# Dane-ME/keypoint-detection

Measured on AMD Instinct MI355X. Metric: images/sec @ 256x192 COCO-17 (MultiPersonKeypointModel.forward, given boxes), higher is better.
Workload: dtype fp32; 1 GPU; C2: batch 64/GPU, 256x192x3, 1 box/img, heatmap head + soft-argmax decode; model=MultiPersonKeypointModel (MobileNetV3-Small+FPN, HeatmapHead), global_batch=64, height=256, width=192, persons=1, precision=split, parallelism=dp1, streams_per_gpu=1, gather=False, gather_pipelined=False

## Files before the change

include/kpd.h:

```cpp
#ifndef KPD_H_
#define KPD_H_

#include <stddef.h>
#include <stdint.h>

#ifdef __cplusplus
extern "C" {
#endif

#define KPD_OK 0
#define KPD_EINVAL (-1)
#define KPD_EHIP (-2)
#define KPD_ESTATE (-3)

#define KPD_PRECISION_FP32 0
#define KPD_PRECISION_MIXED 1
#define KPD_PRECISION_SPLIT 2

typedef struct kpd_plan kpd_plan;

const char* kpd_last_error(void);
const char* kpd_version(void);

int kpd_plan_create(int device, int in_channels, kpd_plan** out);
// ... 115 lines not shown
                              void* stream);

#define KPD_COORD_SMOOTH_L1 0
#define KPD_COORD_MSE 1
#define KPD_COORD_HUBER 2
int kpd_coord_loss(const float* heat, const float* gt, const float* vis, int planes, int H, int W, float temperature,
                   int loss_type, float pixel_weight_scale, float distance_threshold, float* coords, float* loss,
                   float* grad, void* stream);

int kpd_softargmax_backward(const float* heat, const float* grad_coords, int planes, int H, int W, float temperature,
                            float* grad_heat, void* stream);

int kpd_plan_set_streams(kpd_plan* plan, int n);

int kpd_plan_set_graphs(kpd_plan* plan, int enable);

int kpd_bench_conv16(int split, int N, int H, int W, int cin, int cout, int dbg, int iters, float* ms);

#define KPD_BUILD_DIAG 1
int kpd_build_flags(void);

int kpd_fpn0x_class_table(int* cls_ng, int* cls_g, int* cls_woff, int* blocks);


int kpd_heatmap_head(kpd_plan* plan, const float* x, int R, int H, int W, int parts, float* heat, float* ch_w,
                     float* sp_w, void* stream);

int kpd_keypoint_head(kpd_plan* plan, const float* x, int R, int H, int W, float* keypoints, float* visibility,
                      void* stream);

int kpd_backbone(kpd_plan* plan, const float* image, int B, int C, int H, int W, float* out0, float* out1,
                 float* out2, float* out3, void* stream);

int kpd_backbone_body(kpd_plan* plan, const float* image, int B, int C, int H, int W, float* feat0, float* feat1,
                      float* feat2, float* feat3, void* stream);

int kpd_backbone_fpn(kpd_plan* plan, const float* feat0, const float* feat1, const float* feat2, const float* feat3,
                     int B, const int* sizes, float* out0, float* out1, float* out2, float* out3, void* stream);

int kpd_roi_features(kpd_plan* plan, const float* image, int B, int C, int H, int W, const float* boxes, int P,
                     const int32_t* rows, int n, float* out, void* stream);

int kpd_channel_attention(kpd_plan* plan, const float* x, int B, int C, int H, int W, float* scores, int32_t* topk,
                          int k, float* selected, void* stream);

#define KPD_DECODE_ARGMAX 0
// ... 48 lines not shown
```

keypoint-detection_amd/csrc/conv_glds.hip:

```cpp
#include <algorithm>
#include <type_traits>

#include "kpd_common.h"
#include "kpd_kernels.h"
#include "conv_epilogue.h"
#include "kpd_dma.h"

namespace {

typedef _Float16 f16x8 __attribute__((ext_vector_type(8)));
typedef __attribute__((address_space(3))) void lds_void;

constexpr int BM = 256, NT = 512, ROWB = 128;
constexpr unsigned OOB = 0x80000000u;

__device__ __forceinline__ void stamp16(unsigned long long* st, int i, unsigned long long v = 0, int row = -1) {
  if (st && threadIdx.x == 0)
    st[(size_t)(row < 0 ? blockIdx.x : row) * 8 + i] = v ? v : __builtin_amdgcn_s_memrealtime();
}

__device__ __forceinline__ float dpp_xor1(float x) {
  return __int_as_float(__builtin_amdgcn_mov_dpp(__float_as_int(x), 0xB1, 0xF, 0xF, true));
}
__device__ __forceinline__ float dpp_xor2(float x) {
// ... 846 lines not shown
}

constexpr int HP = kHmPitch, HPP = kHmRoiPos;
constexpr int HMS = 56;
constexpr int AWIN = 384;
template <int BMH>
constexpr int hm_awin() { return BMH + 128 <= AWIN ? AWIN : BMH + 128; }
template <int BMH>
constexpr int hm_epi_parts() { return BMH > 256 ? 2 : 1; }
template <int CIN, bool SPLIT>
constexpr int hm_nab() { return (CIN > 0 && (SPLIT ? CIN * 4 : CIN * 2) == 128) ? 1 : 2; }
template <int BMH>
constexpr int kh_epi_parts() { return BMH > 128 ? 2 : 1; }
template <int BN, int BMH>
constexpr int kh_epi_bytes() { return BMH / kh_epi_parts<BMH>() * ((BN + 4) + 68) * 4; }
template <int BN, int SB, int BMH, bool SPLIT, int TPS, int NW, int MODE, int NAB = 2>
constexpr int hmconv_lds_bytes() {
  constexpr int EMODE = MODE >= 0 ? MODE : (BN == 64 ? 1 : 0);
  constexpr int RING = NAB * hm_awin<BMH>() * ROWB + SB * BN * ROWB * TPS;
  constexpr int EPI = EMODE == 2 ? (BN == 128 ? kh_epi_bytes<BN, BMH>() : 0)
                      : EMODE != 0 && EMODE != 3 ? 0 : epi_lds_bytes<BMH / hm_epi_parts<BMH>(), 128, NW * 64>();
  return RING > EPI ? RING : EPI;
}

template <int BMH>
constexpr int hm_pst_stores() { return 2 * 2 * ((BMH / 2 + 31) / 32) * 2; }
template <int BN, int SB, int DBG, int BMH, bool SPLIT, int CIN, int TPS, bool DB, int NW, int MODE, int NTAP,
          bool PST = false>
__device__ __forceinline__ void hmconv_tile(const HmConvArgs& p, char* lds, const int L, const int m_off,
                                            const bool pre = false, const int next_m0 = -1) {
  constexpr int NTH = NW * 64;
  constexpr int EMODE = MODE >= 0 ? MODE : (BN == 64 ? 1 : 0);
  static_assert(NTAP == 9 || (NTAP == 10 && EMODE == 2 && SPLIT && !DB), "tenth tap: KH downsample");
  static_assert(EMODE != 2 || (SPLIT && !DB), "KH epilogue: split, single fragment set");
  constexpr int WAVES_N = BN / 64, WAVES_M = NW / WAVES_N;
  constexpr int WM = BMH / WAVES_M, FM = WM / 16, FN = 4;
  constexpr int AW = hm_awin<BMH>();
  static_assert(WM % 16 == 0 && BMH + 128 <= AW && AW % (8 * NW) == 0, "tile rows");
  static_assert(NW == 8 || (BN == 64 && SPLIT && DB), "4 waves: the conv 3 split DB variant only");
  constexpr int A_LD = AW / 8 / NW;
  static_assert(A_LD <= 9 || TPS > 1, "window pieces: one per tap");
  constexpr int B_LD = BN / 8 / NW;
  constexpr int ABUF = AW * ROWB, BSTAGE = BN * ROWB * TPS;
  static_assert(TPS == 1 || (SPLIT && NTAP % TPS == 0), "taps per step");
  constexpr bool FINAL = EMODE == 1;
  constexpr int NAB = hm_nab<CIN, SPLIT>();
  static_assert(hmconv_lds_bytes<BN, SB, BMH, SPLIT, TPS, NW, MODE, NAB>() <= 160 * 1024, "LDS budget");
  static_assert(!PST || NAB == 2, "persistent tiles: two window buffers");
  static_assert(!PST || (SPLIT && EMODE == 0 && SB == 2 && TPS == 1 && !DB && NW == 8 && NTAP == 9 && BN == 256 &&
                         BMH <= 224 && DBG == 0), "persistent tiles: split conv 1 / conv 2 (BN = cout = 256)");
  auto a_at = [&](int c) { return PST ? (c & 1) * (ABUF + BSTAGE) : NAB == 1 ? 0 : (c & 1) * ABUF; };
  auto b_at = [&](int st) { return PST ? st * (ABUF + BSTAGE) + ABUF : NAB * ABUF + st * BSTAGE; };

  int tid = threadIdx.x;
  if constexpr (PST) asm volatile("" : "+v"(tid));
  const int lane = tid & 63, wave = tid >> 6;
  const int wm = EMODE == 2 ? wave % WAVES_M : wave / WAVES_N, wn = EMODE == 2 ? wave / WAVES_M : wave % WAVES_N;
  const int NTL = p.cout / BN;
  const int m0 = HP + m_off + (L / NTL) * BMH, n0 = (L % NTL) * BN;
  if (m0 >= p.R * HPP) return;
  const int Mtot = p.R * HPP, cin = CIN ? CIN : p.cin, RB = SPLIT ? cin * 4 : cin * 2, NC = RB / 128, KT = NTAP * NC;
  stamp16(p.stamps, 0);
  const int wbase = max(m0 - 64, 0);
  const i32x4 rin = make_rsrc(static_cast<const char*>(p.in) + (size_t)wbase * RB,
                              (int)min(((long)Mtot - wbase) * RB, 0x7fffffffL));
  const i32x4 rwt = make_rsrc(p.wt, p.wt_bytes);
  const unsigned lds0 = (unsigned)reinterpret_cast<unsigned long long>((lds_void*)lds);
  const int lrow = lane >> 3, lchunk = (lane & 7) ^ lrow;
  unsigned a_off[A_LD];
#pragma unroll
  for (int i = 0; i < A_LD; ++i) {
    const int m = m0 - 64 + wave * (AW / NW) + i * 8 + lrow;
    a_off[i] = (m >= 0 && m < Mtot) ? (unsigned)((m - wbase) * RB + lchunk * 16) : OOB;
  }
  unsigned b_off[B_LD];
#pragma unroll
  for (int i = 0; i < B_LD; ++i) {
    const int co = n0 + wave * (BN / NW) + i * 8 + lrow;
    b_off[i] = (unsigned)(co * NTAP * RB + lchunk * 16);
  }
  auto issue_a = [&](int c, int i) {
    const unsigned dst = __builtin_amdgcn_readfirstlane(lds0 + a_at(c) + (wave * (AW / NW) + i * 8) * ROWB);
    glds16(rin, dst, a_off[i] == OOB ? OOB : a_off[i] + c * 128, 0);
  };
  const bool b_dead = EMODE == 2 && SB == 2 && n0 + wave * (BN / NW) >= p.ns + p.nf;
  auto issue_b = [&](int k) {
    if (b_dead) return;
#pragma unroll
    for (int u = 0; u < TPS; ++u) {
      const int sk = k * TPS + u, c = sk / NTAP, t = sk - c * NTAP;
      const unsigned dst = __builtin_amdgcn_readfirstlane(lds0 + b_at(k % SB) + u * BN * ROWB + wave * (BN / NW) * ROWB);
#pragma unroll
      for (int i = 0; i < B_LD; ++i) glds16(rwt, dst + i * 8 * ROWB, b_off[i], t * RB + c * 128);
    }
  };
  static_assert(SB >= 2 && SB <= 4, "weight ring");
  auto barrier_k = [&](bool tail) {
// ... 38 lines not shown
  };
  constexpr int FPRE = (17 * 65 + NTH - 1) / NTH;
  float fin_pre[FPRE];
#pragma unroll
  for (int u = 0; u < FPRE; ++u) fin_pre[u] = 0.f;
  if constexpr (FINAL) {
#pragma unroll
    for (int u = 0; u < FPRE; ++u) {
      const int i = tid + u * NTH;
      if (i < 17 * 64) fin_pre[u] = p.fin_w[i];
      else if (i < 17 * 65) fin_pre[u] = p.fin_b[i - 17 * 64];
    }
  }
  const int rlo = m0 / HPP;
  float us[2] = {1.f, 1.f}, os[2] = {1.f, 1.f};
  if constexpr (SPLIT) {
#pragma unroll
    for (int q = 0; q < 2; ++q) {
      const int rg = p.r0 + min(rlo + q, p.R - 1);
      const float ui = p.in_c + p.in_s * p.hsc[(size_t)rg * 4 + p.in_idx];
      us[q] = ldexpf(1.f, -(split_exp_of(ui) + p.w_exp));
      if (p.out_idx >= 0) os[q] = ldexpf(1.f, split_exp_of(p.out_c + p.out_s * p.hsc[(size_t)rg * 4 + p.out_idx]));
    }
  }
  const int rbound = (rlo + 1) * HPP;
  const int KS = KT / TPS;
  if (!PST || !pre) {
#pragma unroll
    for (int i = 0; i < A_LD; ++i) issue_a(0, i);
#pragma unroll
    for (int k = 0; k < SB - 1; ++k)
      if (k < KS) issue_b(k);
    barrier_k(KS < SB - 1);
  } else {
    if (p.amax_idx >= 0) wait_vmcnt<hm_pst_stores<224>() + 2>();
    else wait_vmcnt<hm_pst_stores<224>()>();
    __builtin_amdgcn_s_waitcnt(0xC07F);
    __builtin_amdgcn_s_barrier();
    asm volatile("" ::: "memory");
  }
  stamp16(p.stamps, 1);
  stamp16(p.stamps, 6, __builtin_amdgcn_s_memtime());
  auto issue_a_at = [&](int k1) {
    const int s1 = k1 * TPS, c1 = s1 / NTAP, jj = (s1 - c1 * NTAP) / TPS;
    if (c1 + 1 >= NC) return;
    if constexpr (TPS == 1) {
      if (jj < A_LD) issue_a(c1 + 1, jj);
    } else {
      constexpr int NST = 9 / TPS;
#pragma unroll
      for (int i = 0; i < A_LD; ++i)
        if (i >= jj * A_LD / NST && i < (jj + 1) * A_LD / NST) issue_a(c1 + 1, i);
    }
  };
  issue_a_at(0);
  if (SB - 1 < KS) issue_b(SB - 1);
  auto issue_at = [&](int k1) {
    if constexpr ((DBG & 2) == 0) {
      issue_a_at(k1);
      if (k1 + SB - 1 < KS) issue_b(k1 + SB - 1);
    }
  };
  if constexpr (!SPLIT) {
    Half f0, f1;
    load_half(0, 0, f0);
    for (int k = 0; k < KT; ++k) {
      load_half(k, 1, f1);
      __builtin_amdgcn_s_setprio(1);
      mma_half(f0);
      __builtin_amdgcn_s_setprio(0);
      if (k + 1 < KT) {
        const int k1 = k + 1;
        barrier_k(k1 + SB - 2 >= KT);
        issue_at(k1);
        load_half(k1, 0, f0);
      } else {
        __builtin_amdgcn_s_waitcnt(0xC07F);
      }
      __builtin_amdgcn_s_setprio(1);
      mma_half(f1);
      __builtin_amdgcn_s_setprio(0);
    }
  } else {
    uint4 ah[FM], al[FM], bh[FN], bl[FN];
    auto rd_a = [&](int k, int q, uint4* f) {
      const int c = k / NTAP, t = k - c * NTAP, off = t == 9 ? 0 : (t / 3 - 1) * HP + (t % 3 - 1);
      const char* ab = lds + a_at(c);
      const int r0w = wm * WM + r16 + 64 + off;
      const int ach = (((q ? 4 : 0) + g) ^ (r0w & 7)) << 4;
#pragma unroll
      for (int i = 0; i < FM; ++i) f[i] = *reinterpret_cast<const uint4*>(ab + (r0w + i * 16) * ROWB + ach);
    };
    const bool late = p.stagger && __builtin_amdgcn_readfirstlane(wave) >= 4;
    auto pass = [&](f32x4 (&A)[FM][FN], const uint4* a, const uint4* b) {
      if constexpr ((DBG & 1) != 0) {
        A[0][0][0] += __uint_as_float(a[0].x ^ b[FN - 1].w);
        return;
      }
      __builtin_amdgcn_s_setprio(1);
#pragma unroll
      for (int i = 0; i < FM; ++i)
#pragma unroll
        for (int j = 0; j < FN; ++j)
          A[i][j] = __builtin_amdgcn_mfma_f32_16x16x32_f16(__builtin_bit_cast(f16x8, a[i]), __builtin_bit_cast(f16x8, b[j]),
                                                           A[i][j], 0, 0, 0);
      __builtin_amdgcn_s_setprio(0);
    };
    if constexpr (DB) {
      static_assert(SB == 2 && 9 % TPS == 0, "DB loop: 2-stage ring");
      int aoff[9];
#pragma unroll
      for (int t = 0; t < 9; ++t) {
        const int r0w = wm * WM + r16 + 64 + (t / 3 - 1) * HP + (t % 3 - 1);
        aoff[t] = r0w * ROWB + ((g ^ (r0w & 7)) << 4);
      }
      struct Frag { uint4 ah[FM], al[FM], bh[FN], bl[FN]; };
// ... 49 lines not shown
        if constexpr (NM_ == FN) {
          pass(A, a, b);
        } else if constexpr (NM_ > 0) {
          if constexpr ((DBG & 1) != 0) {
            A[0][0][0] += __uint_as_float(a[0].x ^ b[0].w);
            return;
          }
          __builtin_amdgcn_s_setprio(1);
#pragma unroll
          for (int i = 0; i < FM; ++i)
#pragma unroll
            for (int j = 0; j < NM_; ++j)
              A[i][j] = __builtin_amdgcn_mfma_f32_16x16x32_f16(__builtin_bit_cast(f16x8, a[i]),
                                                               __builtin_bit_cast(f16x8, b[j]), A[i][j], 0, 0, 0);
          __builtin_amdgcn_s_setprio(0);
        }
      };
      rd_a(0, 1, al);
      rd_bn(0, 0, bh);
      rd_a(0, 0, ah);
      rd_bn(0, 1, bl);
      auto sub = [&](int k, f32x4 (&A)[FM][FN], auto NMx) {
        const bool more = k + 1 < KT, kstep = more && (k + 1) % TPS == 0;
        passn(A, al, bh, NMx);
        if (more) {
          if (kstep) {
            const int k1 = (k + 1) / TPS;
            barrier_k(k1 + SB - 2 >= KS);
            if (!late) issue_at(k1);
          }
          rd_a(k + 1, 1, al);
        }
        passn(A, ah, bh, NMx);
        if (kstep && late) issue_at((k + 1) / TPS);
        if (more) rd_bn(k + 1, 0, bh);
        passn(A, ah, bl, NMx);
        if (more) {
          rd_a(k + 1, 0, ah);
          rd_bn(k + 1, 1, bl);
        }
      };
      if constexpr (NTAP == 10) {
        for (int c = 0; c < NC; ++c) {
          for (int t = 0; t < 9; ++t) sub(c * NTAP + t, acc, NMc);
          sub(c * NTAP + 9, acc2, NM9c);
        }
      } else {
        for (int k = 0; k < KT; ++k) sub(k, acc, NMc);
      }
    };
    using IFN = std::integral_constant<int, FN>;
    if constexpr (EMODE == 2) {
      const int c0 = __builtin_amdgcn_readfirstlane(n0 + wn * 64);
      const int nact = min(max((p.ns + p.nf - c0 + 15) / 16, 0), FN), nact9 = min(max((p.ns - c0 + 15) / 16, 0), FN);
      using I0 = std::integral_constant<int, 0>;
      using I1 = std::integral_constant<int, 1>;
      using I2 = std::integral_constant<int, 2>;
      if (BN == 128 && nact == 2 && nact9 == 0) {
        if constexpr (BN == 128) run_loop(I2{}, I2{}, I0{});
      } else if (BN == 64 && NTAP == 10 && nact == 2 && nact9 == 2) {
        if constexpr (BN == 64 && NTAP == 10) run_loop(I2{}, I2{}, I2{});
      } else if (BN == 64 && NTAP == 9 && nact == 1) {
        if constexpr (BN == 64 && NTAP == 9) run_loop(I1{}, I1{}, I1{});
      } else {
        run_loop(IFN{}, IFN{}, IFN{});
      }
    } else {
      run_loop(IFN{}, IFN{}, IFN{});
    }
    }
  }
  stamp16(p.stamps, 7, __builtin_amdgcn_s_memtime());
  __syncthreads();
  stamp16(p.stamps, 2);
  float pbias[PST ? 2 : 1][8];
  if constexpr (PST) {
#pragma unroll
    for (int h = 0; h < 2; ++h) {
      const int co = n0 + h * 128 + (tid % 16) * 8;
      const float4 b0 = *reinterpret_cast<const float4*>(p.bias + co);
      const float4 b1 = *reinterpret_cast<const float4*>(p.bias + co + 4);
      pbias[h][0] = b0.x; pbias[h][1] = b0.y; pbias[h][2] = b0.z; pbias[h][3] = b0.w;
      pbias[h][4] = b1.x; pbias[h][5] = b1.y; pbias[h][6] = b1.z; pbias[h][7] = b1.w;
    }
    asm volatile("" ::"v"(us[0]), "v"(us[1]), "v"(os[0]), "v"(os[1]));
#pragma unroll
    for (int h = 0; h < 2; ++h)
#pragma unroll
      for (int e = 0; e < 8; ++e) asm volatile("" ::"v"(pbias[h][e]));
    if (next_m0 >= 0) {
      const int nwb = max(next_m0 - 64, 0);
      const i32x4 nrin = make_rsrc(static_cast<const char*>(p.in) + (size_t)nwb * RB,
                                   (int)min(((long)Mtot - nwb) * RB, 0x7fffffffL));
#pragma unroll
      for (int i = 0; i < A_LD; ++i) {
        const int m = next_m0 - 64 + wave * (AW / NW) + i * 8 + lrow;
        const unsigned off = (m >= 0 && m < Mtot) ? (unsigned)((m - nwb) * RB + lchunk * 16) : OOB;
// ... 47 lines not shown
          hi[e] = (_Float16)xs;
          lo[e] = (_Float16)(xs - (float)hi[e]);
        }
        const unsigned off = ok ? (unsigned)((m - m0) * obytes + (co >> 5) * 128 + (co & 31) * 2) : OOB;
        __builtin_amdgcn_raw_buffer_store_b128(__builtin_bit_cast(u32x4, hi), rout, off, 0, 0);
        __builtin_amdgcn_raw_buffer_store_b128(__builtin_bit_cast(u32x4, lo), rout, ok ? off + 64 : OOB, 0, 0);
        if (ok) {
          if (q) mx[1] = fmaxf(mx[1], mc); else mx[0] = fmaxf(mx[0], mc);
        }
      }
    }
    if (p.amax_idx >= 0) {
      const float w0 = wave_max(mx[0]), w1 = wave_max(mx[1]);
      if (lane == 0) {
        const bool two = rlo + 1 < p.R;
        unsigned* a0 = reinterpret_cast<unsigned*>(p.hsc + (size_t)(p.r0 + rlo) * 4 + p.amax_idx);
        unsigned* a1 = reinterpret_cast<unsigned*>(p.hsc + (size_t)(p.r0 + rlo + (two ? 1 : 0)) * 4 + p.amax_idx);
        atomicMax(a0, __float_as_uint(w0));
        atomicMax(a1, __float_as_uint(two ? w1 : 0.f));
      }
    }
  } else if constexpr (EMODE == 0 || EMODE == 3) {
    float* tile = reinterpret_cast<float*>(lds);
    constexpr int RP = hm_epi_parts<BMH>(), BR = BMH / RP, WPR = WAVES_M / RP;
    static_assert(WAVES_M % RP == 0, "epilogue row parts");
    constexpr int P4 = 128 + 4, C8 = 16, RS = NTH / C8, IT = (BR + RS - 1) / RS;
    __bf16* out = reinterpret_cast<__bf16*>(p.out);
    float mx[2] = {0.f, 0.f};
#pragma unroll
    for (int ph = 0; ph < RP * (BN / 128); ++ph) {
      const int pr = ph / (BN / 128), h = ph % (BN / 128);
      if (ph) __syncthreads();
      if (wn / 2 == h && wm / WPR == pr) acc_to_lds<FM, FN, WM, 64, 128>(tile, acc, wm % WPR, wn % 2, lane);
      __syncthreads();
      const int c8 = tid % C8, row0 = tid / C8, co = n0 + h * 128 + c8 * 8;
      const float4 b0 = *reinterpret_cast<const float4*>(p.bias + co);
      const float4 b1 = *reinterpret_cast<const float4*>(p.bias + co + 4);
      const float bv[8] = {b0.x, b0.y, b0.z, b0.w, b1.x, b1.y, b1.z, b1.w};
#pragma unroll
      for (int it = 0; it < IT; ++it) {
        const int row = row0 + it * RS, m = m0 + pr * BR + row;
        int r, yy, xx;
        if (row >= BR || !interior(m, r, yy, xx)) continue;
        const float4 x0 = *reinterpret_cast<const float4*>(tile + row * P4 + c8 * 8);
        const float4 x1 = *reinterpret_cast<const float4*>(tile + row * P4 + c8 * 8 + 4);
        float xv[8] = {x0.x, x0.y, x0.z, x0.w, x1.x, x1.y, x1.z, x1.w};
        if constexpr (EMODE == 3) {
          const float u = m >= rbound ? us[1] : us[0];
// ... 245 lines not shown
            o[e] = x;
          }
          if (co < p.ns) {
            const float sc = q ? os[1] : os[0];
            f16x4 hi, lo;
  #pragma unroll
            for (int e = 0; e < 4; ++e) {
              const float xs = o[e] * sc;
              hi[e] = (_Float16)xs;
              lo[e] = (_Float16)(xs - (float)hi[e]);
            }
            char* ob = static_cast<char*>(p.out) + (size_t)m * (p.ns * 4) + (co >> 5) * 128 + (co & 31) * 2;
            *reinterpret_cast<f16x4*>(ob) = hi;
            *reinterpret_cast<f16x4*>(ob + 64) = lo;
          } else {
            *reinterpret_cast<float4*>(p.outf + ((size_t)r * HMS * HMS + yy * HMS + xx) * p.nf +
                                       (co - p.ns)) = make_float4(o[0], o[1], o[2], o[3]);
          }
        }
      }
  
    }
  }
  if (p.stamps) {
    asm volatile("s_waitcnt vmcnt(0)" ::: "memory");
    stamp16(p.stamps, 3);
    stamp16(p.stamps, 5, (unsigned long long)KT);
  }
}

template <int BN, int SB, int DBG = 0, int BMH = BM, bool SPLIT = false, int CIN = 0, int TPS = 1, bool DB = false,
          int NW = 8, int MODE = -1, int NTAP = 9>
__global__ __launch_bounds__(NW * 64) void hmconv_kernel(const HmConvArgs p) {
  __shared__ __attribute__((aligned(1024))) char lds[hmconv_lds_bytes<BN, SB, BMH, SPLIT, TPS, NW, MODE,
                                                                      hm_nab<CIN, SPLIT>()>()];
  hmconv_tile<BN, SB, DBG, BMH, SPLIT, CIN, TPS, DB, NW, MODE, NTAP>(p, lds, xcd_remap(blockIdx.x, gridDim.x),
                                                                        p.m_off);
}

template <typename T>
__device__ __forceinline__ void kernarg_copy(T& dst) {
  typedef const __attribute__((address_space(4))) unsigned* KaPtr;
  KaPtr ka = (KaPtr)__builtin_amdgcn_kernarg_segment_ptr();
  asm volatile("" : "+s"(ka));
  static_assert(sizeof(T) % 4 == 0, "argument block");
  unsigned* d = reinterpret_cast<unsigned*>(&dst);
#pragma unroll
  for (int i = 0; i < (int)(sizeof(T) / 4); ++i) d[i] = ka[i];
}

template <int CIN>
__global__ __launch_bounds__(512) void hmconv_persist_kernel(const HmConvArgs p) {
  __shared__ __attribute__((aligned(1024))) char lds[hmconv_lds_bytes<256, 2, 224, true, 1, 8, -1>()];
  const int G = gridDim.x, w = xcd_remap(blockIdx.x, G);
  const int F = p.mix_F, H = p.mix_H, tail_off = p.m_off + F * 224;
  bool pre = false;
  for (int t = w; t < F; t += G) {
    HmConvArgs pl;
    kernarg_copy(pl);
    const int nt = t + G;
// ... 11 lines not shown

template <int BN, int SB, int BMH, int BMT, int CIN, int TPS, bool DB, int MODE>
__global__ __launch_bounds__(512) void hmconv_mixed_kernel(const HmConvArgs p) {
  constexpr int LB = hmconv_lds_bytes<BN, SB, BMH, true, TPS, 8, MODE>(),
                LT = hmconv_lds_bytes<BN, SB, BMT, true, TPS, 8, MODE>();
  __shared__ __attribute__((aligned(1024))) char lds[LB > LT ? LB : LT];
  const int x = blockIdx.x % 8, k = blockIdx.x / 8;
  const int Fx = p.mix_F / 8, Hx = p.mix_H / 8, h0 = min(Hx, p.mix_lead);
  bool tail;
  int idx;
  if (k < 2 * h0) {
    tail = (k & 1) == 0;
    idx = k >> 1;
  } else if (k - 2 * h0 < Fx - h0) {
    tail = false;
    idx = h0 + (k - 2 * h0);
  } else {
    tail = true;
    idx = h0 + (k - 2 * h0 - (Fx - h0));
  }
  if (tail) hmconv_tile<BN, SB, 0, BMT, true, CIN, TPS, DB, 8, MODE, 9>(p, lds, x * Hx + idx,
                                                                       p.m_off + (p.mix_F / (p.cout / BN)) * BMH);
  else hmconv_tile<BN, SB, 0, BMH, true, CIN, TPS, DB, 8, MODE, 9>(p, lds, x * Fx + idx, p.m_off);
}

constexpr long kMaxDesc = 0x7fffffffL;

template <bool SPLIT, typename TO, int KS, int BN, int S, bool PF = (BN <= 128)>
hipError_t launch(const Conv16Args& a0, hipStream_t st) {
  constexpr long OS = sizeof(TO);
  Conv16Args a = a0;
  const long wt_bytes = (long)a.cout_p * KS * KS * a.cin_e * 2;
  const long HW = (long)a.H * a.W;
  const long img_bytes = HW * a.in_cstride * 2;
  if (wt_bytes > kMaxDesc || img_bytes > kMaxDesc) return hipErrorInvalidValue;
  a.wt_bytes = (int)wt_bytes;
  const int chunk = (int)std::min<long>(a.N, kMaxDesc / img_bytes);
  for (int n0 = 0; n0 < a0.N; n0 += chunk) {
    const int nb = std::min(chunk, a0.N - n0);
    a.N = nb;
    a.M = (int)(nb * HW);
    a.in = static_cast<const char*>(a0.in) + n0 * img_bytes;
    a.out = static_cast<char*>(a0.out) + n0 * HW * a.out_cstride * OS;
    a.stats = a0.stats ? a0.stats + (long)n0 * a.tiles_per_img * 2 * a.cout_p : nullptr;
    a.in_bytes = (int)(nb * img_bytes);
    a.r0 = a0.r0 + n0;
// ... 218 lines not shown
        const hipError_t e = hipGetLastError();
        if (e != hipSuccess) return e;
        continue;
      }
    }
    static const bool no_tail12 = kpd_diag_env("KPD_HM12_NOTAIL") != nullptr;
#if KPD_DIAG
    static const int persist_env = kpd_diag_env("KPD_HM_PERSIST") ? atoi(kpd_diag_env("KPD_HM_PERSIST")) : 0;
    if (split && !fin && bn == 256 && bm == 224 && a.cout == 256 && (a.cin == 64 || a.cin == 256) && !dbg &&
        !a.stamps && persist_env) {
      const long F = rows / 224 / ncu * ncu, rem = rows - F * 224, H = (rem + 191) / 192;
      if (F > 0 && H <= ncu && F + H < 0x7fffffffL / 224) {
        HmConvArgs m = a;
        m.mix_F = (int)F;
        m.mix_H = (int)H;
        if (a.cin == 64) hipLaunchKernelGGL((hmconv_persist_kernel<64>), dim3((unsigned)ncu), dim3(NT), 0, st, m);
        else hipLaunchKernelGGL((hmconv_persist_kernel<256>), dim3((unsigned)ncu), dim3(NT), 0, st, m);
        const hipError_t e = hipGetLastError();
        if (e != hipSuccess) return e;
        continue;
      }
    }
#endif
    const long F12 = rows / 224 / ncu * ncu, rem12 = rows - F12 * 224;
    const bool t160 = (rem12 + 159) / 160 <= ncu;
    const long H12 = t160 ? (rem12 + 159) / 160 : (rem12 + 191) / 192;
    if (split && !fin && bn == 256 && bm == 224 && (a.cin == 64 || a.cin == 256) && !dbg && !a.stamps) {
      if (mix_ok(F12, H12)) {
        HmConvArgs m = a;
        dim3 g;
        mix_set(m, F12, H12, g);
        if (a.cin == 64 && t160) hipLaunchKernelGGL((hmconv_mixed_kernel<256, 2, 224, 160, 64, 1, false, -1>), g, dim3(NT), 0, st, m);
        else if (a.cin == 64) hipLaunchKernelGGL((hmconv_mixed_kernel<256, 2, 224, 192, 64, 1, false, -1>), g, dim3(NT), 0, st, m);
        else if (t160) hipLaunchKernelGGL((hmconv_mixed_kernel<256, 2, 224, 160, 256, 1, false, -1>), g, dim3(NT), 0, st, m);
        else hipLaunchKernelGGL((hmconv_mixed_kernel<256, 2, 224, 192, 256, 1, false, -1>), g, dim3(NT), 0, st, m);
        const hipError_t e = hipGetLastError();
        if (e != hipSuccess) return e;
        continue;
      }
    }
    if (split && !fin && bn == 256 && bm == 224 && a.cin == 256 && !dbg && !no_tail12 && !a.stamps) {
      if (F12 > 0 && rem12 > 0 && H12 <= ncu) {
        const dim3 g1((unsigned)F12), g2((unsigned)H12);
        HmConvArgs a2 = a;
        a2.m_off = (int)(F12 * 224);
        hipLaunchKernelGGL((hmconv_kernel<256, 2, 0, 224, true, 256>), g1, dim3(NT), 0, st, a);
// ... 157 lines not shown
```

keypoint-detection_amd/csrc/kpd_kernels.h:

```cpp
#pragma once
#include <hip/hip_runtime.h>
#include <stdint.h>
#include <vector>

struct ConvArgs {
  const void* in;
  const void* wt;
  const float* bias;
  void* out;
  const float* res;
  const float* a_scale;
  float* stats;
  int N, H, W;
  int cin_p, cout_p;
  int in_cstride, out_cstride;
  int rh, rw;
  int act;
  int M;
  int tiles_per_img;
  float* amax;
  const float* post_scale;
  const float* post_shift;
  int act2, act3;
  int in_bytes, wt_bytes;
// ... 34 lines not shown
  int in_idx;
  float out_c, out_s;
  int out_idx;
  int amax_idx;
  int w_exp;
  const float *fin_w, *fin_b;
  const int32_t* slot;
  int P;
  float* heat;
  int r0;
  int m_off;
  int mix_F, mix_H, mix_lead;
  int in_bytes, wt_bytes;
  int stagger;
  unsigned long long* stamps;
  const float *kh_ps, *kh_pt, *kh_bd;
  float* outf;
  int ns, nf, ntap;
};
hipError_t launch_hmconv(const HmConvArgs& a, hipStream_t st);
constexpr int kHmPitch = 57, kHmRoiPos = kHmPitch * kHmPitch;
__host__ __device__ inline size_t hm_pos(size_t r, int y, int x) {
  return r * kHmRoiPos + (size_t)(y + 1) * kHmPitch + x;
}

constexpr int kFpn0xMaxGroups = 4;
constexpr int kFpn0xMaxImg = 512;
constexpr int kFpn0xPairFirst[16] = {-1, -1, 1, -1, -1, -1, -1, -1, 4, 5, 6, 7, -1, -1, 13, -1};
constexpr unsigned kFpn0xSecondMask = 1u << 2 | 1u << 8 | 1u << 9 | 1u << 10 | 1u << 11 | 1u << 14;
constexpr unsigned kFpn0xFirstMask = 1u << 1 | 1u << 4 | 1u << 5 | 1u << 6 | 1u << 7 | 1u << 13;
constexpr unsigned kFpn0xSlot(int c0, int c1, int c2) { return (unsigned)(c0 | c1 << 5 | c2 << 10); }
constexpr unsigned kFpn0xSlots[8] = {kFpn0xSlot(5, 9, 0),    kFpn0xSlot(1, 2, 31),   kFpn0xSlot(3, 31, 31),
                                     kFpn0xSlot(4, 8, 31),   kFpn0xSlot(6, 10, 12),  kFpn0xSlot(13, 14, 31),
                                     kFpn0xSlot(15, 31, 31), kFpn0xSlot(7, 11, 31)};
constexpr unsigned kFpn0xSlots10[10] = {kFpn0xSlot(5, 9, 31),   kFpn0xSlot(0, 31, 31),  kFpn0xSlot(1, 2, 31),
                                        kFpn0xSlot(3, 31, 31),  kFpn0xSlot(4, 8, 31),   kFpn0xSlot(6, 10, 31),
                                        kFpn0xSlot(12, 31, 31), kFpn0xSlot(13, 14, 31), kFpn0xSlot(15, 31, 31),
                                        kFpn0xSlot(7, 11, 31)};
struct Fpn0xArgs {
  const void* f_split;
  const void* l_split;
  const void* w0;
  const void* weff;
  int cls_woff[16];
  int cls_ng[16];
  int cls_g[16][kFpn0xMaxGroups];
// ... 305 lines not shown
```

keypoint-detection_amd/csrc/kpd_pack.hip:

```cpp
#include "kpd_plan_int.h"

namespace {

int se_squeeze(int c) {
  const int v = c / 4;
  int n = std::max(8, (int)(v + 4) / 8 * 8);
  if (n < 0.9 * v) n += 8;
  return n;
}

uint16_t f2bf(float f) {
  uint32_t u;
  std::memcpy(&u, &f, 4);
  if ((u & 0x7fffffffu) > 0x7f800000u) return (uint16_t)((u >> 16) | 0x40);
  u += 0x7fffu + ((u >> 16) & 1u);
  return (uint16_t)(u >> 16);
}

const HostT* get(kpd_plan* p, const std::string& name, std::string& missing) {
  auto it = p->t.find(name);
  if (it == p->t.end()) {
    missing += name + " ";
    return nullptr;
  }
// ... 314 lines not shown
                     hE.data() + p->fpn0x.cls_woff[cls]);
  }
  if (int rc = upload(p, h0, &p->fpn0x.w0)) return rc;
  if (int rc = upload(p, hE, &p->fpn0x.weff)) return rc;
  p->fpn0x.w0_bytes = (int)(h0.size() * 2);
  p->fpn0x.weff_bytes = (int)(hE.size() * 2);
  p->fpn0x.w_exp0 = e0;
  p->fpn0x.w_expE = eE;
  return KPD_OK;
}

}

extern "C" {

int kpd_fpn0x_class_table(int* cls_ng, int* cls_g, int* cls_woff, int* blocks) {
  if (!cls_ng || !cls_g || !cls_woff || !blocks) return fail(KPD_EINVAL, "NULL output");
  const int nb = fpn0x_class_table(cls_ng, reinterpret_cast<int(*)[kFpn0xMaxGroups]>(cls_g), cls_woff);
  if (nb < 0) return fail(KPD_ESTATE, "fpn0x: inconsistent class table");
  *blocks = nb;
  return KPD_OK;
}

int kpd_plan_finalize(kpd_plan* p, int precision) {
  if (!p) return fail(KPD_EINVAL, "null plan");
  if (precision != KPD_PRECISION_FP32 && precision != KPD_PRECISION_MIXED && precision != KPD_PRECISION_SPLIT)
    return fail(KPD_EINVAL, "unknown precision");
  HIP_TRY(hipSetDevice(p->device));
  for (void* a : p->allocs) (void)hipFree(a);
  p->allocs.clear();
  p->fpn0x.w0 = p->fpn0x.weff = nullptr;
  p->stamps = nullptr;
  p->pd = DevConv();
  p->anchors = nullptr;
  p->hm1 = DevConv();
  p->hm2 = DevConv();
  p->hm3 = DevConv();
  for (auto& c : p->fpn_lv) c = DevConv();
  p->kh_ds1 = DevConv();
  p->kh_ds2 = DevConv();
  for (auto& k : p->kh_s) k = KhSplit();
  p->kh_split = false;
  p->has_kh = false;
  for (int k = 0; k <= kpd_plan::kMaxSub; ++k) {
    if (p->ws[k]) { (void)hipFree(p->ws[k]); p->ws[k] = nullptr; p->ws_bytes[k] = 0; }
    p->have_work[k] = false;
// ... 213 lines not shown
```

keypoint-detection_amd/dll/_native.py:

```python
from __future__ import annotations

import ctypes
import os
from pathlib import Path
from typing import List, Optional

import torch

_LIB_PATH = Path(__file__).resolve().parent / "_lib" / "libkpd.so"
_lib: Optional[ctypes.CDLL] = None

KPD_PRECISION_FP32 = 0
KPD_PRECISION_MIXED = 1
KPD_PRECISION_SPLIT = 2
PRECISIONS = {"fp32": KPD_PRECISION_FP32, "split": KPD_PRECISION_SPLIT, "mixed": KPD_PRECISION_MIXED,
              "bf16": KPD_PRECISION_MIXED}

EXPORTS = ("kpd_last_error", "kpd_version", "kpd_plan_create", "kpd_plan_set_tensor",
           "kpd_plan_finalize", "kpd_plan_destroy", "kpd_forward", "kpd_debug_copy", "kpd_nms",
           "kpd_plan_timing", "kpd_plan_timing_stage", "kpd_plan_timing_query", "kpd_plan_set_detector",
           "kpd_bench_conv16", "kpd_build_flags", "kpd_fpn0x_class_table",
           "kpd_plan_set_streams", "kpd_preprocess", "kpd_target_heatmaps", "kpd_keypoint_metrics",
           "kpd_heatmap_head", "kpd_keypoint_head", "kpd_backbone", "kpd_channel_attention", "kpd_decode_heatmaps",
           "kpd_roi_align", "kpd_conv1x1", "kpd_adaptive_heatmap_loss", "kpd_conv3x3_forward",
           "kpd_conv3x3_backward", "kpd_conv3x3_forward_prec", "kpd_conv3x3_backward_prec", "kpd_plan_set_graphs", "kpd_backbone_body", "kpd_backbone_fpn",
           "kpd_plan_path_log", "kpd_plan_path_query", "kpd_preprocess_batch", "kpd_draw_poses",
           "kpd_oks_match", "kpd_pose_nms", "kpd_flip_merge", "kpd_augment_batch", "kpd_bn_train_forward",
           "kpd_bn_train_backward", "kpd_roi_targets", "kpd_roi_features", "kpd_detector_features",
           "kpd_detector_targets", "kpd_detector_loss", "kpd_coord_loss", "kpd_softargmax_backward")
PRE_BATCH_CHUNK = 32
DRAW_BOXES, DRAW_LIMBS, DRAW_JOINTS, DRAW_HEAT = 1, 2, 4, 8
DRAW_CHUNK = 32
DRAW_TILE_W = 64
DRAW_TILE_H = 16
DRAW_MAX_SIDE = 16384
DRAW_MAX_WIDTH = 512
DRAW_MAX_HEAT = 1024
OKS_MAX_K = 32
OKS_MAX_T = 16
OKS_MAX_D = 64
OKS_MAX_G = 64
POSE_NMS_MAX_D = 64
POSE_NMS_MAX_K = 32
POSE_NMS_HARD, POSE_NMS_SOFT, POSE_NMS_SOFT_LINEAR = 0, 1, 2
# ... 60 lines not shown
    lib.kpd_plan_path_query.argtypes = [c_void_p, c_char_p, ctypes.c_size_t, ctypes.POINTER(ctypes.c_size_t)]
    lib.kpd_target_heatmaps.argtypes = [c_void_p, c_int, c_int, c_int, ctypes.c_double, c_void_p, c_void_p]
    lib.kpd_keypoint_metrics.argtypes = [c_void_p, c_void_p, c_void_p, ctypes.c_long, ctypes.POINTER(ctypes.c_float),
                                         c_int, c_void_p, c_void_p]
    lib.kpd_preprocess_batch.argtypes = [ctypes.POINTER(c_void_p), ctypes.POINTER(c_int), ctypes.POINTER(c_int),
                                         ctypes.POINTER(c_int), c_int, c_int, c_int, ctypes.c_float, c_int, c_int,
                                         c_int, c_int, ctypes.POINTER(ctypes.c_float),
                                         ctypes.POINTER(ctypes.c_float), c_void_p, c_void_p]
    u8p = ctypes.POINTER(ctypes.c_uint8)
    lib.kpd_draw_poses.argtypes = [ctypes.POINTER(c_void_p), ctypes.POINTER(c_int), ctypes.POINTER(c_int),
                                   ctypes.POINTER(c_int), c_int, c_void_p, c_void_p, c_void_p, c_void_p,
                                   c_int, c_int, c_int, c_int, ctypes.POINTER(c_int), c_int, u8p, u8p, u8p,
                                   c_int, c_int, c_int, c_int, c_int, c_int, c_int, c_void_p]
    lib.kpd_oks_match.argtypes = [c_void_p] * 8 + [ctypes.POINTER(ctypes.c_float)] * 2 + [c_int] * 6 + \
        [c_void_p] * 8
    lib.kpd_pose_nms.argtypes = [c_void_p] * 5 + [ctypes.POINTER(ctypes.c_float)] + [c_int] * 4 + \
        [ctypes.c_float] * 3 + [c_int] + [c_void_p] * 6
    lib.kpd_flip_merge.argtypes = [c_void_p] * 3 + [ctypes.POINTER(ctypes.c_int32)] + [c_int] * 5 + [c_void_p] * 5
    i32p = ctypes.POINTER(ctypes.c_int32)
    lib.kpd_augment_batch.argtypes = [ctypes.POINTER(c_void_p)] + [ctypes.POINTER(c_int)] * 3 + \
        [ctypes.POINTER(c_void_p), c_int, c_int, i32p, ctypes.POINTER(ctypes.c_double), ctypes.POINTER(c_int),
         i32p, i32p, u8p, i32p, c_void_p, c_void_p, c_void_p, c_int, c_int, c_void_p, c_void_p, c_void_p, c_void_p]
    lib.kpd_fpn0x_class_table.argtypes = [ctypes.POINTER(c_int)] * 4
    lib.kpd_nms.argtypes = [c_void_p, c_void_p, c_int, ctypes.c_float, c_int, c_void_p, c_void_p, c_void_p]
    c_float = ctypes.c_float
    lib.kpd_heatmap_head.argtypes = [c_void_p, c_void_p, c_int, c_int, c_int, c_int, c_void_p, c_void_p, c_void_p,
                                     c_void_p]
    lib.kpd_keypoint_head.argtypes = [c_void_p, c_void_p, c_int, c_int, c_int, c_void_p, c_void_p, c_void_p]
    lib.kpd_backbone.argtypes = [c_void_p, c_void_p, c_int, c_int, c_int, c_int, c_void_p, c_void_p, c_void_p,
                                 c_void_p, c_void_p]
    lib.kpd_backbone_body.argtypes = [c_void_p, c_void_p, c_int, c_int, c_int, c_int, c_void_p, c_void_p, c_void_p,
                                      c_void_p, c_void_p]
    lib.kpd_backbone_fpn.argtypes = [c_void_p, c_void_p, c_void_p, c_void_p, c_void_p, c_int,
                                     ctypes.POINTER(c_int), c_void_p, c_void_p, c_void_p, c_void_p, c_void_p]
    lib.kpd_channel_attention.argtypes = [c_void_p, c_void_p, c_int, c_int, c_int, c_int, c_void_p, c_void_p, c_int,
                                          c_void_p, c_void_p]
    lib.kpd_decode_heatmaps.argtypes = [c_void_p, c_int, c_int, c_int, c_int, c_float, c_void_p, c_void_p, c_void_p,
                                        c_void_p]
    lib.kpd_roi_align.argtypes = [c_void_p, c_int, c_int, c_int, c_int, c_void_p, c_int, c_int, c_int, c_float, c_int,
                                  c_int, c_void_p, c_void_p]
    lib.kpd_conv1x1.argtypes = [c_void_p, c_int, c_int, c_int, c_void_p, c_void_p, c_int, c_void_p, c_void_p]
    lib.kpd_adaptive_heatmap_loss.argtypes = [c_void_p, c_void_p, c_void_p, c_int, c_int, c_int, c_int, c_float,
                                              c_float, c_int, c_float, c_void_p, c_void_p, c_void_p, c_void_p]
    lib.kpd_conv3x3_forward.argtypes = [c_void_p, c_void_p, c_void_p, c_int, c_int, c_int, c_int, c_int, c_void_p,
                                        c_void_p]
    lib.kpd_conv3x3_backward.argtypes = [c_void_p, c_void_p, c_void_p, c_int, c_int, c_int, c_int, c_int, c_void_p,
# ... 638 lines not shown
```

Measured before the change: 42650 images/s.

## Add pair-tile heatmap conv kernels splitting 256-wide tiles into two 128-column halves

Adds a 4-wave, 128-column "pair" variant of the split-precision heatmap 3x3 conv. It uses a single shared A window of reduced size, loads the window in three staged pieces across the taps, and fits in about 80KB of LDS so two blocks can be resident per CU. The cin=64 conv with cout 256 and BM 224 now launches twice as many half-width tiles by default, optionally as a mixed full/tail grid. The aim is higher occupancy and better latency hiding on the first head conv, at the cost of reloading the A window once per half and adding more barriers.

```diff
diff --git a/include/kpd.h b/include/kpd.h
--- a/include/kpd.h
+++ b/include/kpd.h
@@ -161,6 +161,8 @@
 
 int kpd_fpn0x_class_table(int* cls_ng, int* cls_g, int* cls_woff, int* blocks);
 
+int kpd_hmconv_row_geometry(int rois, int ncu, long long* full_tiles, int* tail_rows, long long* tail_tiles);
+
 
 int kpd_heatmap_head(kpd_plan* plan, const float* x, int R, int H, int W, int parts, float* heat, float* ch_w,
                      float* sp_w, void* stream);
diff --git a/keypoint-detection_amd/csrc/conv_glds.hip b/keypoint-detection_amd/csrc/conv_glds.hip
--- a/keypoint-detection_amd/csrc/conv_glds.hip
+++ b/keypoint-detection_amd/csrc/conv_glds.hip
@@ -892,6 +892,14 @@
                       : EMODE != 0 && EMODE != 3 ? 0 : epi_lds_bytes<BMH / hm_epi_parts<BMH>(), 128, NW * 64>();
   return RING > EPI ? RING : EPI;
 }
+constexpr int kHmPairWin = 352;
+constexpr int kHmPairs = 1;
+constexpr bool kHmPairMix = true;
+constexpr bool hm_is_pair(int BN, int NW, bool SPLIT, int EMODE) { return BN == 128 && NW == 4 && SPLIT && EMODE == 0; }
+constexpr int hm_pair_lds_bytes() {
+  constexpr int RING = kHmPairWin * ROWB + 2 * 128 * ROWB, EPI = epi_lds_bytes<112, 128, 256>();
+  return RING > EPI ? RING : EPI;
+}
 
 template <int BMH>
 constexpr int hm_pst_stores() { return 2 * 2 * ((BMH / 2 + 31) / 32) * 2; }
@@ -905,23 +913,28 @@
   static_assert(EMODE != 2 || (SPLIT && !DB), "KH epilogue: split, single fragment set");
   constexpr int WAVES_N = BN / 64, WAVES_M = NW / WAVES_N;
   constexpr int WM = BMH / WAVES_M, FM = WM / 16, FN = 4;
-  constexpr int AW = hm_awin<BMH>();
+  constexpr bool PAIR = hm_is_pair(BN, NW, SPLIT, EMODE);
+  static_assert(!PAIR || (SB == 2 && TPS == 1 && !DB && NTAP == 9 && !PST && BMH <= 224 && DBG == 0),
+                "pair tiles: split conv 1 / conv 2 halves");
+  constexpr int AW = PAIR ? kHmPairWin : hm_awin<BMH>();
   static_assert(WM % 16 == 0 && BMH + 128 <= AW && AW % (8 * NW) == 0, "tile rows");
-  static_assert(NW == 8 || (BN == 64 && SPLIT && DB), "4 waves: the conv 3 split DB variant only");
+  static_assert(NW == 8 || (BN == 64 && SPLIT && DB) || PAIR, "4 waves: the conv 3 split DB variant and pair tiles");
   constexpr int A_LD = AW / 8 / NW;
-  static_assert(A_LD <= 9 || TPS > 1, "window pieces: one per tap");
+  static_assert(A_LD <= 9 || TPS > 1 || PAIR, "window pieces: one per tap (PAIR: by dead row range)");
   constexpr int B_LD = BN / 8 / NW;
   constexpr int ABUF = AW * ROWB, BSTAGE = BN * ROWB * TPS;
   static_assert(TPS == 1 || (SPLIT && NTAP % TPS == 0), "taps per step");
   constexpr bool FINAL = EMODE == 1;
-  constexpr int NAB = hm_nab<CIN, SPLIT>();
-  static_assert(hmconv_lds_bytes<BN, SB, BMH, SPLIT, TPS, NW, MODE, NAB>() <= 160 * 1024, "LDS budget");
+  constexpr int NAB = PAIR ? 1 : hm_nab<CIN, SPLIT>();
+  static_assert(PAIR ? hm_pair_lds_bytes() <= 80 * 1024 && ABUF + 2 * BSTAGE <= hm_pair_lds_bytes()
+                     : hmconv_lds_bytes<BN, SB, BMH, SPLIT, TPS, NW, MODE, NAB>() <= 160 * 1024, "LDS budget");
   static_assert(!PST || NAB == 2, "persistent tiles: two window buffers");
   static_assert(!PST || (SPLIT && EMODE == 0 && SB == 2 && TPS == 1 && !DB && NW == 8 && NTAP == 9 && BN == 256 &&
                          BMH <= 224 && DBG == 0), "persistent tiles: split conv 1 / conv 2 (BN = cout = 256)");
   auto a_at = [&](int c) { return PST ? (c & 1) * (ABUF + BSTAGE) : NAB == 1 ? 0 : (c & 1) * ABUF; };
   auto b_at = [&](int st) { return PST ? st * (ABUF + BSTAGE) + ABUF : NAB * ABUF + st * BSTAGE; };
 
+  unsigned long long* const stamps = PAIR ? nullptr : p.stamps;
   int tid = threadIdx.x;
   if constexpr (PST) asm volatile("" : "+v"(tid));
   const int lane = tid & 63, wave = tid >> 6;
@@ -930,19 +943,38 @@
   const int m0 = HP + m_off + (L / NTL) * BMH, n0 = (L % NTL) * BN;
   if (m0 >= p.R * HPP) return;
   const int Mtot = p.R * HPP, cin = CIN ? CIN : p.cin, RB = SPLIT ? cin * 4 : cin * 2, NC = RB / 128, KT = NTAP * NC;
-  stamp16(p.stamps, 0);
+  stamp16(stamps, 0);
   const int wbase = max(m0 - 64, 0);
   const i32x4 rin = make_rsrc(static_cast<const char*>(p.in) + (size_t)wbase * RB,
                               (int)min(((long)Mtot - wbase) * RB, 0x7fffffffL));
   const i32x4 rwt = make_rsrc(p.wt, p.wt_bytes);
   const unsigned lds0 = (unsigned)reinterpret_cast<unsigned long long>((lds_void*)lds);
   const int lrow = lane >> 3, lchunk = (lane & 7) ^ lrow;
-  unsigned a_off[A_LD];
-#pragma unroll
-  for (int i = 0; i < A_LD; ++i) {
-    const int m = m0 - 64 + wave * (AW / NW) + i * 8 + lrow;
-    a_off[i] = (m >= 0 && m < Mtot) ? (unsigned)((m - wbase) * RB + lchunk * 16) : OOB;
-  }
+  unsigned a_off[PAIR ? 1 : A_LD];
+  if constexpr (!PAIR) {
+#pragma unroll
+    for (int i = 0; i < A_LD; ++i) {
+      const int m = m0 - 64 + wave * (AW / NW) + i * 8 + lrow;
+      a_off[i] = (m >= 0 && m < Mtot) ? (unsigned)((m - wbase) * RB + lchunk * 16) : OOB;
+    }
+  }
+  constexpr int NPC = (BMH + 122 + 7) / 8;
+  static_assert(!PAIR || NPC * 8 <= AW, "pair window");
+  const int ws = __builtin_amdgcn_readfirstlane(wave);
+  auto hw_lane = [] { return (int)__builtin_amdgcn_mbcnt_hi(~0u, __builtin_amdgcn_mbcnt_lo(~0u, 0u)); };
+  auto issue_ap = [&](int c, int lo, int hi) {
+    int ln = hw_lane();
+    asm volatile("" : "+v"(ln));
+    const int lr = ln >> 3, row = m0 - 64 + lr, boff = (m0 - 64 - wbase + lr) * RB + ((ln & 7) ^ lr) * 16 + c * 128;
+#pragma unroll
+    for (int i = 0; i < A_LD; ++i) {
+      const int gp = i * NW + ws;
+      if (gp >= lo && gp < hi) {
+        const unsigned off = (unsigned)(row + gp * 8) < (unsigned)Mtot ? (unsigned)(boff + gp * 8 * RB) : OOB;
+        glds16(rin, __builtin_amdgcn_readfirstlane(lds0 + gp * 8 * ROWB), off, 0);
+      }
+    }
+  };
   unsigned b_off[B_LD];
 #pragma unroll
   for (int i = 0; i < B_LD; ++i) {
@@ -1027,12 +1059,23 @@
       us[q] = ldexpf(1.f, -(split_exp_of(ui) + p.w_exp));
       if (p.out_idx >= 0) os[q] = ldexpf(1.f, split_exp_of(p.out_c + p.out_s * p.hsc[(size_t)rg * 4 + p.out_idx]));
     }
+    if constexpr (PAIR) {
+#pragma unroll
+      for (int q = 0; q < 2; ++q) {
+        us[q] = __uint_as_float(__builtin_amdgcn_readfirstlane(__float_as_uint(us[q])));
+        os[q] = __uint_as_float(__builtin_amdgcn_readfirstlane(__float_as_uint(os[q])));
+      }
+    }
   }
   const int rbound = (rlo + 1) * HPP;
   const int KS = KT / TPS;
   if (!PST || !pre) {
-#pragma unroll
-    for (int i = 0; i < A_LD; ++i) issue_a(0, i);
+    if constexpr (PAIR) {
+      issue_ap(0, 0, NPC);
+    } else {
+#pragma unroll
+      for (int i = 0; i < A_LD; ++i) issue_a(0, i);
+    }
 #pragma unroll
     for (int k = 0; k < SB - 1; ++k)
       if (k < KS) issue_b(k);
@@ -1044,12 +1087,15 @@
     __builtin_amdgcn_s_barrier();
     asm volatile("" ::: "memory");
   }
-  stamp16(p.stamps, 1);
-  stamp16(p.stamps, 6, __builtin_amdgcn_s_memtime());
+  stamp16(stamps, 1);
+  stamp16(stamps, 6, __builtin_amdgcn_s_memtime());
   auto issue_a_at = [&](int k1) {
     const int s1 = k1 * TPS, c1 = s1 / NTAP, jj = (s1 - c1 * NTAP) / TPS;
     if (c1 + 1 >= NC) return;
-    if constexpr (TPS == 1) {
+    if constexpr (PAIR) {
+      if (jj == 3) issue_ap(c1 + 1, 0, 7);
+      else if (jj == 6) issue_ap(c1 + 1, 7, 15);
+    } else if constexpr (TPS == 1) {
       if (jj < A_LD) issue_a(c1 + 1, jj);
     } else {
       constexpr int NST = 9 / TPS;
@@ -1096,7 +1142,7 @@
 #pragma unroll
       for (int i = 0; i < FM; ++i) f[i] = *reinterpret_cast<const uint4*>(ab + (r0w + i * 16) * ROWB + ach);
     };
-    const bool late = p.stagger && __builtin_amdgcn_readfirstlane(wave) >= 4;
+    const bool late = !PAIR && p.stagger && __builtin_amdgcn_readfirstlane(wave) >= 4;
     auto pass = [&](f32x4 (&A)[FM][FN], const uint4* a, const uint4* b) {
       if constexpr ((DBG & 1) != 0) {
         A[0][0][0] += __uint_as_float(a[0].x ^ b[FN - 1].w);
@@ -1192,12 +1238,19 @@
       rd_bn(0, 1, bl);
       auto sub = [&](int k, f32x4 (&A)[FM][FN], auto NMx) {
         const bool more = k + 1 < KT, kstep = more && (k + 1) % TPS == 0;
+        const bool cb = PAIR && more && (k + 1) % 9 == 0;
         passn(A, al, bh, NMx);
         if (more) {
           if (kstep) {
             const int k1 = (k + 1) / TPS;
             barrier_k(k1 + SB - 2 >= KS);
             if (!late) issue_at(k1);
+          }
+          if constexpr (PAIR) {
+            if (cb) {
+              issue_ap((k + 1) / 9, 15, NPC);
+              barrier_k(true);
+            }
           }
           rd_a(k + 1, 1, al);
         }
@@ -1240,9 +1293,10 @@
     }
     }
   }
-  stamp16(p.stamps, 7, __builtin_amdgcn_s_memtime());
+  stamp16(stamps, 7, __builtin_amdgcn_s_memtime());
   __syncthreads();
-  stamp16(p.stamps, 2);
+  stamp16(stamps, 2);
+  const int tid_k = tid, lane_k = lane, wave_k = wave, wm_k = wm, wn_k = wn;
   float pbias[PST ? 2 : 1][8];
   if constexpr (PST) {
 #pragma unroll
@@ -1336,8 +1390,16 @@
     }
   } else if constexpr (EMODE == 0 || EMODE == 3) {
     float* tile = reinterpret_cast<float*>(lds);
-    constexpr int RP = hm_epi_parts<BMH>(), BR = BMH / RP, WPR = WAVES_M / RP;
+    int tid = tid_k;
+    if constexpr (PAIR) {
+      tid = ws * 64 + hw_lane();
+      asm volatile("" : "+v"(tid));
+    }
+    const int lane = PAIR ? (tid & 63) : lane_k, wave = PAIR ? (tid >> 6) : wave_k;
+    const int wm = PAIR ? wave / WAVES_N : wm_k, wn = PAIR ? wave % WAVES_N : wn_k;
+    constexpr int RP = PAIR ? 2 : hm_epi_parts<BMH>(), BR = BMH / RP, WPR = WAVES_M / RP;
     static_assert(WAVES_M % RP == 0, "epilogue row parts");
+    static_assert(!PAIR || (BR * (128 + 4) + 2 * NW) * 4 <= hm_pair_lds_bytes(), "pair epilogue stage");
     constexpr int P4 = 128 + 4, C8 = 16, RS = NTH / C8, IT = (BR + RS - 1) / RS;
     __bf16* out = reinterpret_cast<__bf16*>(p.out);
     float mx[2] = {0.f, 0.f};
@@ -1629,10 +1691,10 @@
   
     }
   }
-  if (p.stamps) {
+  if (stamps) {
     asm volatile("s_waitcnt vmcnt(0)" ::: "memory");
-    stamp16(p.stamps, 3);
-    stamp16(p.stamps, 5, (unsigned long long)KT);
+    stamp16(stamps, 3);
+    stamp16(stamps, 5, (unsigned long long)KT);
   }
 }
 
@@ -1643,6 +1705,12 @@
                                                                       hm_nab<CIN, SPLIT>()>()];
   hmconv_tile<BN, SB, DBG, BMH, SPLIT, CIN, TPS, DB, NW, MODE, NTAP>(p, lds, xcd_remap(blockIdx.x, gridDim.x),
                                                                         p.m_off);
+}
+
+template <int BMH, int CIN>
+__global__ __launch_bounds__(256, 2) void hmconv_pair_kernel(const HmConvArgs p) {
+  __shared__ __attribute__((aligned(1024))) char lds[hm_pair_lds_bytes()];
+  hmconv_tile<128, 2, 0, BMH, true, CIN, 1, false, 4, 0, 9>(p, lds, xcd_remap(blockIdx.x, gridDim.x), p.m_off);
 }
 
 template <typename T>
@@ -1700,6 +1768,27 @@
   if (tail) hmconv_tile<BN, SB, 0, BMT, true, CIN, TPS, DB, 8, MODE, 9>(p, lds, x * Hx + idx,
                                                                        p.m_off + (p.mix_F / (p.cout / BN)) * BMH);
   else hmconv_tile<BN, SB, 0, BMH, true, CIN, TPS, DB, 8, MODE, 9>(p, lds, x * Fx + idx, p.m_off);
+}
+
+template <int BMT, int CIN>
+__global__ __launch_bounds__(256, 2) void hmconv_pair_mixed_kernel(const HmConvArgs p) {
+  __shared__ __attribute__((aligned(1024))) char lds[hm_pair_lds_bytes()];
+  const int x = blockIdx.x % 8, k = blockIdx.x / 8;
+  const int Fx = p.mix_F / 8, Hx = p.mix_H / 8, h0 = min(Hx, p.mix_lead);
+  bool tail;
+  int idx;
+  if (k < 2 * h0) {
+    tail = (k & 1) == 0;
+    idx = k >> 1;
+  } else if (k - 2 * h0 < Fx - h0) {
+    tail = false;
+    idx = h0 + (k - 2 * h0);
+  } else {
+    tail = true;
+    idx = h0 + (k - 2 * h0 - (Fx - h0));
+  }
+  if (tail) hmconv_tile<128, 2, 0, BMT, true, CIN, 1, false, 4, 0, 9>(p, lds, x * Hx + idx, p.m_off + (p.mix_F / 2) * 224);
+  else hmconv_tile<128, 2, 0, 224, true, CIN, 1, false, 4, 0, 9>(p, lds, x * Fx + idx, p.m_off);
 }
 
 constexpr long kMaxDesc = 0x7fffffffL;
@@ -1964,6 +2053,50 @@
       }
     }
 #endif
+    int pairs = kHmPairs;
+    bool pair_mix = kHmPairMix;
+#if KPD_DIAG
+    static const int pairs_env = kpd_diag_env("KPD_HM_PAIRS") ? atoi(kpd_diag_env("KPD_HM_PAIRS")) : kHmPairs;
+    static const int pmix_env = kpd_diag_env("KPD_HM_PAIR_MIX") ? atoi(kpd_diag_env("KPD_HM_PAIR_MIX")) : -1;
+    pairs = pairs_env;
+    if (pmix_env >= 0) pair_mix = pmix_env != 0;
+#endif
+    if (split && !fin && bn == 256 && bm == 224 && a.cout == 256 && !dbg && !a.stamps &&
+        ((a.cin == 64 && (pairs & 1)) || (a.cin == 256 && (pairs & 2) && KPD_DIAG))) {
+      const HmRowGeometry geo = hm_row_geometry(nr, ncu);
+      if (geo.full + geo.tail < 0x7fffffffL / 224 / 2) {
+        const dim3 g1((unsigned)(2 * geo.full)), g2((unsigned)(2 * geo.tail));
+        if (pair_mix && a.cin == 64 && geo.tail > 0 && ncu % 8 == 0) {
+          HmConvArgs m = a;
+          m.mix_F = (int)(2 * geo.full);
+          m.mix_H = (int)((2 * geo.tail + 7) / 8 * 8);
+          m.mix_lead = ncu / 8;
+          const dim3 g((unsigned)(m.mix_F + m.mix_H));
+          if (geo.tail_rows == 160) hipLaunchKernelGGL((hmconv_pair_mixed_kernel<160, 64>), g, dim3(256), 0, st, m);
+          else hipLaunchKernelGGL((hmconv_pair_mixed_kernel<192, 64>), g, dim3(256), 0, st, m);
+          const hipError_t e = hipGetLastError();
+          if (e != hipSuccess) return e;
+          continue;
+        }
+        HmConvArgs a2 = a;
+        a2.m_off = (int)(geo.full * 224);
+        if (a.cin == 64) {
+          hipLaunchKernelGGL((hmconv_pair_kernel<224, 64>), g1, dim3(256), 0, st, a);
+          if (geo.tail_rows == 160) hipLaunchKernelGGL((hmconv_pair_kernel<160, 64>), g2, dim3(256), 0, st, a2);
+          else if (geo.tail_rows == 192) hipLaunchKernelGGL((hmconv_pair_kernel<192, 64>), g2, dim3(256), 0, st, a2);
+        }
+#if KPD_DIAG
+        else {
+          hipLaunchKernelGGL((hmconv_pair_kernel<224, 256>), g1, dim3(256), 0, st, a);
+          if (geo.tail_rows == 160) hipLaunchKernelGGL((hmconv_pair_kernel<160, 256>), g2, dim3(256), 0, st, a2);
+          else if (geo.tail_rows == 192) hipLaunchKernelGGL((hmconv_pair_kernel<192, 256>), g2, dim3(256), 0, st, a2);
+        }
+#endif
+        const hipError_t e = hipGetLastError();
+        if (e != hipSuccess) return e;
+        continue;
+      }
+    }
     const long F12 = rows / 224 / ncu * ncu, rem12 = rows - F12 * 224;
     const bool t160 = (rem12 + 159) / 160 <= ncu;
     const long H12 = t160 ? (rem12 + 159) / 160 : (rem12 + 191) / 192;
diff --git a/keypoint-detection_amd/csrc/kpd_kernels.h b/keypoint-detection_amd/csrc/kpd_kernels.h
--- a/keypoint-detection_amd/csrc/kpd_kernels.h
+++ b/keypoint-detection_amd/csrc/kpd_kernels.h
@@ -80,6 +80,19 @@
 constexpr int kHmPitch = 57, kHmRoiPos = kHmPitch * kHmPitch;
 __host__ __device__ inline size_t hm_pos(size_t r, int y, int x) {
   return r * kHmRoiPos + (size_t)(y + 1) * kHmPitch + x;
+}
+struct HmRowGeometry {
+  long full;
+  int tail_rows;
+  long tail;
+};
+inline HmRowGeometry hm_row_geometry(long rois, int ncu) {
+  const long rows = rois * kHmRoiPos - kHmPitch, F = rows / 224 / ncu * ncu, rem = rows - F * 224;
+  if (F > 0 && rem > 0) {
+    if ((rem + 159) / 160 <= ncu) return {F, 160, (rem + 159) / 160};
+    if ((rem + 191) / 192 <= ncu) return {F, 192, (rem + 191) / 192};
+  }
+  return {(rows + 223) / 224, 0, 0};
 }
 
 constexpr int kFpn0xMaxGroups = 4;
diff --git a/keypoint-detection_amd/csrc/kpd_pack.hip b/keypoint-detection_amd/csrc/kpd_pack.hip
--- a/keypoint-detection_amd/csrc/kpd_pack.hip
+++ b/keypoint-detection_amd/csrc/kpd_pack.hip
@@ -360,6 +360,16 @@
   return KPD_OK;
 }
 
+int kpd_hmconv_row_geometry(int rois, int ncu, long long* full_tiles, int* tail_rows, long long* tail_tiles) {
+  if (!full_tiles || !tail_rows || !tail_tiles) return fail(KPD_EINVAL, "NULL output");
+  if (rois <= 0 || ncu <= 0) return fail(KPD_EINVAL, "rois and ncu must be positive");
+  const HmRowGeometry g = hm_row_geometry(rois, ncu);
+  *full_tiles = g.full;
+  *tail_rows = g.tail_rows;
+  *tail_tiles = g.tail;
+  return KPD_OK;
+}
+
 int kpd_plan_finalize(kpd_plan* p, int precision) {
   if (!p) return fail(KPD_EINVAL, "null plan");
   if (precision != KPD_PRECISION_FP32 && precision != KPD_PRECISION_MIXED && precision != KPD_PRECISION_SPLIT)
diff --git a/keypoint-detection_amd/dll/_native.py b/keypoint-detection_amd/dll/_native.py
--- a/keypoint-detection_amd/dll/_native.py
+++ b/keypoint-detection_amd/dll/_native.py
@@ -19,7 +19,7 @@
 EXPORTS = ("kpd_last_error", "kpd_version", "kpd_plan_create", "kpd_plan_set_tensor",
            "kpd_plan_finalize", "kpd_plan_destroy", "kpd_forward", "kpd_debug_copy", "kpd_nms",
            "kpd_plan_timing", "kpd_plan_timing_stage", "kpd_plan_timing_query", "kpd_plan_set_detector",
-           "kpd_bench_conv16", "kpd_build_flags", "kpd_fpn0x_class_table",
+           "kpd_bench_conv16", "kpd_build_flags", "kpd_fpn0x_class_table", "kpd_hmconv_row_geometry",
            "kpd_plan_set_streams", "kpd_preprocess", "kpd_target_heatmaps", "kpd_keypoint_metrics",
            "kpd_heatmap_head", "kpd_keypoint_head", "kpd_backbone", "kpd_channel_attention", "kpd_decode_heatmaps",
            "kpd_roi_align", "kpd_conv1x1", "kpd_adaptive_heatmap_loss", "kpd_conv3x3_forward",
@@ -126,6 +126,8 @@
         [ctypes.POINTER(c_void_p), c_int, c_int, i32p, ctypes.POINTER(ctypes.c_double), ctypes.POINTER(c_int),
          i32p, i32p, u8p, i32p, c_void_p, c_void_p, c_void_p, c_int, c_int, c_void_p, c_void_p, c_void_p, c_void_p]
     lib.kpd_fpn0x_class_table.argtypes = [ctypes.POINTER(c_int)] * 4
+    lib.kpd_hmconv_row_geometry.argtypes = [c_int, c_int, ctypes.POINTER(ctypes.c_longlong), ctypes.POINTER(c_int),
+                                            ctypes.POINTER(ctypes.c_longlong)]
     lib.kpd_nms.argtypes = [c_void_p, c_void_p, c_int, ctypes.c_float, c_int, c_void_p, c_void_p, c_void_p]
     c_float = ctypes.c_float
     lib.kpd_heatmap_head.argtypes = [c_void_p, c_void_p, c_int, c_int, c_int, c_int, c_void_p, c_void_p, c_void_p,
```

New measurement: 42970 images/s (median of 6 runs). No clear change (+0.7%).
